# ownzonefeng/pytorch-distributed-training-example

Hardware: AMD Instinct MI355X
Metric: images/sec (whole node) ResNet-50 DDP at 1/2/4/8 MI355X; scaling efficiency (higher is better)
Workload: dtype bf16; 1 GPU; model=resnet50, global_batch=1024, per_gpu_batch=1024, image_size=224, parallelism=dp1, grad_accum=1, impl=ours, graph=False, precision=bf16, bucket_cap_mb=auto, comm_hook=none, reducer_active=True, pg_size=1, pg_backend=nccl, deterministic=False, full=False

## Files before the change

### pytorch_distributed_training_example_amd/config.py

```python
from __future__ import annotations

import os


class _Switches:
    __slots__ = ("disable_native", "conv1x1", "conv1x1_ours", "conv1x1_prefer", "conv1x1_override",
                 "conv1x1_table", "conv1x1_dump", "conv1x1_s2", "conv3x3", "conv3x3_wgrad", "conv3x3_s2", "conv_stem",
                 "conv_bn_stats", "bn_bwd_stats", "res_masked", "stem_bwd_fused", "stem_bn_wgrad", "stem_bn_stats", "stem_pool_wgrad", "wgrad_splitk", "slice_sum",
                 "subsample_native", "linear_splitk", "fused_addln", "embedding_native", "linear_epilogue",
                 "bwd_fused", "bwd_fused_shapes", "bwd_alg", "alg_glo", "bwd_alg_min_m", "z3_virtual", "bwd_alg_first", "ds_alg", "bn2_defer", "bn_apply_gemm_k", "strided_bstats", "gap_native", "sub_out",
                 "fp8_fused_gelu", "fp8_weight_multi", "fp8_cast_colsum", "fp8_ln", "wgrad_stream_m",
                 "dropout_fused")

    def __init__(self):
        self.reload()

    def reload(self) -> "_Switches":
        e = os.environ.get

        def on(name: str, default: str = "1") -> bool:
            return e(name, default) != "0"

        self.disable_native = e("PDT_DISABLE_NATIVE", "0") == "1"
        self.conv1x1 = e("PDT_CONV1X1", "auto")
# ... 2 lines not shown
        ov = e("PDT_CONV1X1_OVERRIDE", "")
        self.conv1x1_override = dict(p.split("=", 1) for p in ov.replace("+", ";").split(";") if "=" in p)
        self.conv1x1_table = on("PDT_CONV1X1_TABLE")
        self.conv1x1_dump = e("PDT_CONV1X1_DUMP") or None
        self.conv1x1_s2 = e("PDT_CONV1X1_S2", "1") == "1"
        self.conv3x3 = e("PDT_CONV3X3", "ours")
        self.conv3x3_wgrad = e("PDT_CONV3X3_WGRAD", "ours")
        self.conv3x3_s2 = e("PDT_CONV3X3_S2", "ours")
        self.conv_stem = e("PDT_CONV_STEM", "ours")
        self.conv_bn_stats = on("PDT_CONV_BN_STATS")
        self.bn_bwd_stats = on("PDT_BN_BWD_STATS")
        self.res_masked = on("PDT_RES_MASKED")
        self.stem_bwd_fused = on("PDT_STEM_BWD_FUSED")
        self.stem_bn_wgrad = on("PDT_STEM_BN_WGRAD")
        self.stem_bn_stats = on("PDT_STEM_BN_STATS")
        self.stem_pool_wgrad = on("PDT_STEM_POOL_WGRAD")
        self.wgrad_splitk = on("PDT_WGRAD_SPLITK")
        self.slice_sum = on("PDT_SLICE_SUM")
        self.subsample_native = on("PDT_SUBSAMPLE_NATIVE")
        self.linear_splitk = on("PDT_LINEAR_SPLITK")
        self.fused_addln = on("PDT_FUSED_ADDLN")
        self.embedding_native = on("PDT_EMBEDDING_NATIVE")
        self.linear_epilogue = e("PDT_LINEAR_EPILOGUE", "auto")
        self.bwd_fused = on("PDT_BWD_FUSED")
        self.bwd_fused_shapes = tuple(tuple(int(v) for v in t.split("x")) for t in
                                      e("PDT_BWD_FUSED_SHAPES", "256x64").split(",") if "x" in t)
        self.bwd_alg = int(e("PDT_BWD_ALG", "2"))
        self.bwd_alg_min_m = int(e("PDT_BWD_ALG_MIN_M", "50176"))
        self.alg_glo = on("PDT_ALG_GLO", "1")
        self.z3_virtual = int(e("PDT_Z3_VIRTUAL", "2"))
        self.bwd_alg_first = on("PDT_BWD_ALG_FIRST", "1")
        self.ds_alg = int(e("PDT_DS_ALG", "512"))
        self.bn2_defer = on("PDT_BN2_DEFER", "0")
        self.bn_apply_gemm_k = int(e("PDT_BN_APPLY_GEMM_K", "128"))
        self.strided_bstats = on("PDT_STRIDED_BSTATS")
        self.gap_native = on("PDT_GAP_NATIVE")
        self.sub_out = on("PDT_SUB_OUT")
        self.fp8_fused_gelu = on("PDT_FP8_FUSED_GELU")
        self.fp8_weight_multi = on("PDT_FP8_WEIGHT_MULTI")
        self.fp8_cast_colsum = on("PDT_FP8_CAST_COLSUM")
        self.fp8_ln = on("PDT_FP8_LN")
        self.wgrad_stream_m = int(e("PDT_WGRAD_STREAM_M", "0"))
        self.dropout_fused = on("PDT_DROPOUT_FUSED")
        return self


SW = _Switches()
```

### pytorch_distributed_training_example_amd/csrc/binding.cpp

```cpp
#include <torch/extension.h>
#include <ATen/hip/HIPContext.h>

#include <cstring>
#include <map>
#include <vector>

#include "fp8_pack.h"
#include "launchers.h"

namespace {

using at::Tensor;

hipStream_t stream() { return at::hip::getCurrentHIPStream().stream(); }

int dcode(const Tensor& t) {
  if (t.scalar_type() == at::kFloat) return 0;
  if (t.scalar_type() == at::kBFloat16) return 1;
  TORCH_CHECK(false, "pdt: unsupported dtype ", t.scalar_type(), " (fp32 / bf16 only)");
}

void check_cuda(const Tensor& t, const char* name) {
  TORCH_CHECK(t.is_cuda(), "pdt: ", name, " must be a GPU tensor");
}
// ... 2291 lines not shown
  m.doc() = "gfx950 HIP kernels for pytorch_distributed_training_example_amd";
  m.def("sgd", &sgd);
  m.def("adam", &adam);
  m.def("adadelta", &adadelta);
  m.def("lars", &lars);
  m.def("lamb", &lamb);
  m.def("layerwise_chunks", &layerwise_chunks);
  m.def("amp_unscale", &amp_unscale);
  m.def("amp_update", &amp_update);
  m.def("mt_scale", &mt_scale);
  m.def("mt_copy", &mt_copy);
  m.def("l2norm_sq", &l2norm_sq);
  m.def("clip_coef", &clip_coef);
  m.def("bn_tune", [](int variant, int target_blocks, int u_fwd, int u_bwd) {
    if (pdt_bn_tune(variant, target_blocks, u_fwd, u_bwd) != 0)
      throw py::value_error("bn_tune: variant must be 0 (keep), 3 (in-kernel finalize) or 5 (finalize kernel), got " +
                            std::to_string(variant));
  }, py::arg("variant") = 0, py::arg("target_blocks") = 0, py::arg("u_fwd") = 0, py::arg("u_bwd") = 0);
  m.def("bn_fwd_train", &bn_fwd_train, py::arg("x"), py::arg("res"), py::arg("weight"), py::arg("bias"),
        py::arg("running_mean"), py::arg("running_var"), py::arg("momentum"), py::arg("eps"), py::arg("relu"),
        py::arg("res_ab") = py::none(), py::arg("apply") = true);
  m.def("bn_fwd_eval", &bn_fwd_eval);
  m.def("bn_relu_maxpool_fwd", &bn_relu_maxpool_fwd);
  m.def("bn_relu_maxpool_fwd_parts", &bn_relu_maxpool_fwd_parts);
  m.def("maxpool3s2_bwd", &maxpool3s2_bwd);
  m.def("conv1x1_gemm", &conv1x1_gemm, py::arg("a"), py::arg("b"), py::arg("out"), py::arg("acc"), py::arg("stats"),
        py::arg("c_in") = py::none(), py::arg("c_mask") = py::none(), py::arg("bn_x") = py::none(),
        py::arg("bn_mask") = py::none(), py::arg("bn_mean") = py::none(), py::arg("c_stride") = 0,
        py::arg("c_H") = 0, py::arg("c_W") = 0, py::arg("a_coef") = py::none(), py::arg("bn_sum_only") = false,
        py::arg("no_store") = false);
  m.def("conv1x1_probe", [](int probe) { pdt_conv1x1_probe(probe); });
  m.def("conv1x1_persist", [](int mode) { return pdt_conv1x1_persist(mode); },
        "1x1 GEMM persistence mode (0 off, 1 measured kinds, 2 all, -1 env default); returns the previous mode");
  m.def("conv1x1_last_persistent", []() { return pdt_conv1x1_last_persistent(); },
        "which kernel the last 1x1 GEMM call launched: 0 one tile per workgroup, else the persistent kernel's waves "
        "per workgroup (+256 statistics-only, +512 APPLY)");
  m.def("conv3x3_opt", [](int v) { return pdt_conv3x3_opt(v); },
        "3x3 conv variant bits (csrc/kernels/conv3x3.hip conv3x3_opt; -1 env default); returns the previous value");
  m.def("weight_prep", &weight_prep);
  m.def("bn_tiles_fused", [](int on) { pdt_bn_tiles_fused(on); });
  m.def("maxpool_bwd_v2", [](int on) { pdt_maxpool_bwd_v2(on); });
  m.def("pool_fwd_contig", [](int on) { pdt_pool_fwd_contig(on); });
  m.def("bn_apply_wgs", [](int n) { pdt_bn_apply_wgs(n); });
  m.def("bn_row_wgs", [](int n) { pdt_bn_row_wgs(n); });
  m.def("gap_bwd", &gap_bwd, py::arg("g"), py::arg("H"), py::arg("W"), py::arg("bn_x") = py::none(),
        py::arg("bn_mask") = py::none(), py::arg("bn_mean") = py::none(), py::arg("bn_sum_only") = false);
  m.def("conv1x1_gemm_apply", &conv1x1_gemm_apply, py::arg("a"), py::arg("b"), py::arg("res"), py::arg("ab"),
        py::arg("rab") = py::none(), py::arg("a_coef") = py::none());
  m.def("bn_bwd_train_tiles", &bn_bwd_train_tiles);
  m.def("maxpool3s2_bwd_bn", &maxpool3s2_bwd_bn);
  m.def("maxpool3s2_bwd_bn_coef", &maxpool3s2_bwd_bn_coef, py::arg("dy"), py::arg("code"), py::arg("x"),
        py::arg("weight"), py::arg("mean"), py::arg("invstd"), py::arg("need_dgamma"), py::arg("write_dz") = true);
  m.def("slice_sum", &slice_sum);
  m.def("subsample_gather", &subsample_gather);
  m.def("subsample_scatter_add", &subsample_scatter_add);
  m.def("bn_fwd_train_tiles", &bn_fwd_train_tiles, py::arg("x"), py::arg("part"), py::arg("res"), py::arg("weight"),
        py::arg("bias"), py::arg("running_mean"), py::arg("running_var"), py::arg("momentum"), py::arg("eps"),
        py::arg("relu"), py::arg("res_ab") = py::none(), py::arg("apply") = true, py::arg("sub") = 0);
  m.def("conv3x3s1_fwd", &conv3x3s1_fwd);
  m.def("conv3x3s1_fwd_stats", &conv3x3s1_fwd_stats);
  m.def("conv3x3s1_fwd_bnbwd", &conv3x3s1_fwd_bnbwd);
  m.def("conv3x3_flip", &conv3x3_flip);
  m.def("conv3x3s2_fwd", &conv3x3s2_fwd);
  m.def("conv3x3s2_wgrad", &conv3x3s2_wgrad);
  m.def("conv3x3s2_dgrad", &conv3x3s2_dgrad, py::arg("dy"), py::arg("wf"), py::arg("H"), py::arg("W"),
        py::arg("bn_x") = py::none(), py::arg("bn_mask") = py::none(), py::arg("bn_mean") = py::none());
// ... 93 lines not shown
```

### pytorch_distributed_training_example_amd/csrc/kernels/conv1x1.hip

```cpp
#include "../common.h"
#include "../launchers.h"
#include "../tile_stats.h"

#include <stdlib.h>

using namespace pdt;

namespace {

typedef __bf16 bf16x8 __attribute__((ext_vector_type(8)));
typedef float f4 __attribute__((ext_vector_type(4)));
#define PDT_LDS __attribute__((address_space(3)))

__device__ __attribute__((aligned(256))) uint4 g_gemm_zero[16];
__device__ __attribute__((aligned(256))) uint4 g_gemm_ones[16] = {
    {0x3f803f80u, 0x3f803f80u, 0x3f803f80u, 0x3f803f80u}, {0x3f803f80u, 0x3f803f80u, 0x3f803f80u, 0x3f803f80u},
    {0x3f803f80u, 0x3f803f80u, 0x3f803f80u, 0x3f803f80u}, {0x3f803f80u, 0x3f803f80u, 0x3f803f80u, 0x3f803f80u},
    {0x3f803f80u, 0x3f803f80u, 0x3f803f80u, 0x3f803f80u}, {0x3f803f80u, 0x3f803f80u, 0x3f803f80u, 0x3f803f80u},
    {0x3f803f80u, 0x3f803f80u, 0x3f803f80u, 0x3f803f80u}, {0x3f803f80u, 0x3f803f80u, 0x3f803f80u, 0x3f803f80u},
    {0x3f803f80u, 0x3f803f80u, 0x3f803f80u, 0x3f803f80u}, {0x3f803f80u, 0x3f803f80u, 0x3f803f80u, 0x3f803f80u},
    {0x3f803f80u, 0x3f803f80u, 0x3f803f80u, 0x3f803f80u}, {0x3f803f80u, 0x3f803f80u, 0x3f803f80u, 0x3f803f80u},
    {0x3f803f80u, 0x3f803f80u, 0x3f803f80u, 0x3f803f80u}, {0x3f803f80u, 0x3f803f80u, 0x3f803f80u, 0x3f803f80u},
    {0x3f803f80u, 0x3f803f80u, 0x3f803f80u, 0x3f803f80u}, {0x3f803f80u, 0x3f803f80u, 0x3f803f80u, 0x3f803f80u}};
__device__ uint8_t g_mask_ones[16] = {
// ... 310 lines not shown
      v.z = (uint32_t)f2bf(z[4]) | ((uint32_t)f2bf(z[5]) << 16);
      v.w = (uint32_t)f2bf(z[6]) | ((uint32_t)f2bf(z[7]) << 16);
    }
    if constexpr (BSTATS) {
      bn_bwd_accum8(v, xbv[it], bmkv[it], bmu, bs1, bs2);
      v = mask8(v, bmkv[it]);
    }
    if (!ok) continue;
    if constexpr (STATS) rs8_add(rst, v);
    if constexpr (APPLY) {
      if (!(probe & 32)) ap.mask[off >> 3] = (uint8_t)amb;
    }
    if constexpr (!NOST) {
      if (probe & 1) continue;
      if constexpr (NT) {
        const u32x4 t = {v.x, v.y, v.z, v.w};
        __builtin_nontemporal_store(t, reinterpret_cast<u32x4*>(Y + off));
      } else {
        *reinterpret_cast<uint4*>(Y + off) = v;
      }
    }
  }
  }

  if constexpr (BSTATS)
    bn_bwd_tile_store<BN, Cf::kWaves>(bs1, bs2, reinterpret_cast<float*>(lds), bs.part, (M + BM - 1) / BM, mt, N, n0);
  if constexpr (STATS) {
    __syncthreads();
    rs8_tile_store<BN, Cf::kWaves>(rst, kst, reinterpret_cast<float*>(lds), part, min(BM, M - m0), (M + BM - 1) / BM,
                                   mt, N, n0);
  }
}

template <class Cf, int HV = 0>
struct PL {
  static constexpr int kStgOff = 2 * Cf::kSlot;
  static constexpr int kFull = Cf::BM * Cf::kEpiStride;
  static constexpr int kHalves = HV > 0 ? HV : (kStgOff + kFull <= 152 * 1024 ? 1 : 2);
  static_assert(Cf::WM % kHalves == 0, "a part is whole wave rows");
  static constexpr int kStg = kFull / kHalves;
  static constexpr int kRed0 = Cf::kWaves * (Cf::BN / 8) * 16 * 4, kRed1 = Cf::kWaves * 2 * Cf::BN * 4;
  static constexpr int kRed = kRed0 > kRed1 ? kRed0 : kRed1;
  static constexpr int kArea = kStg > kRed ? kStg : kRed;
  static constexpr int kLds = 3 * Cf::kSlot > kStgOff + kArea ? 3 * Cf::kSlot : kStgOff + kArea;
  static constexpr int kOcc = (160 * 1024) / kLds;
  static constexpr int kMinWaves = kOcc * Cf::kThreads / 256 > 0 ? kOcc * Cf::kThreads / 256 : 1;
  static_assert(kLds <= 160 * 1024 && kFull % kHalves == 0, "LDS");
};

__device__ __attribute__((aligned(256))) uint4 g_gemm_sink[1024];
__device__ uint8_t g_mask_sink[1024];

__device__ __forceinline__ void dma16a(const void* src, char* lds_wave_base) {
  const uint32_t m0 = __builtin_amdgcn_readfirstlane((uint32_t)(uintptr_t)(PDT_LDS const char*)lds_wave_base);
  asm volatile("s_mov_b32 m0, %1\n\ts_nop 0\n\tglobal_load_lds_dwordx4 %0, off" ::"v"(src), "s"(m0) : "memory");
}
template <int N>
__device__ __forceinline__ void wait_vmn() {
  static_assert(N >= 0 && N < 64, "vmcnt");
  __builtin_amdgcn_s_waitcnt((N & 15) | (7 << 4) | (15 << 8) | ((N >> 4) << 14));
}

template <class Cf, bool ACC, bool STATS, bool BSTATS, bool ATR, bool APPLY, bool STR, bool NOST = false, int HV = 0>
__global__ __launch_bounds__(Cf::kThreads, (PL<Cf, HV>::kMinWaves)) void conv1x1p_kernel(
    const uint16_t* __restrict__ A, const uint16_t* __restrict__ B, uint16_t* Y, const uint16_t* Cin,
    const uint8_t* __restrict__ Cmask, float* __restrict__ part, int M, int K, int N, BnSrc bs, CGeom cg,
    const float* __restrict__ acoef, ApArgs ap) {
  static_assert(!(APPLY && (ACC || STATS || BSTATS)), "APPLY is a forward epilogue of its own");
  static_assert(!STR || ACC, "STR: a strided accumulate source");
  static_assert(!NOST || (STATS && !ACC && !BSTATS && !APPLY), "NOST: the statistics-only forward");
  using L = PL<Cf, HV>;
  constexpr int BM = Cf::BM, BN = Cf::BN, kG = Cf::kG, kHalves = L::kHalves;
  constexpr int WROWS = BM / Cf::WM, WCOLS = BN / Cf::WN;
  extern __shared__ __attribute__((aligned(16))) char lds[];
  const int tid = threadIdx.x, lane = tid & 63, wid = __builtin_amdgcn_readfirstlane(tid >> 6);
  const int wm = wid % Cf::WM, wn = wid / Cf::WM;
  const int ntn = N / BN, T = (M + BM - 1) / BM, total = T * ntn;
  const int G = gridDim.x, xg = blockIdx.x % 8, jg = blockIdx.x / 8, gx = (G - xg + 7) / 8;
  const int c_lo = (int)((int64_t)total * xg / 8), c_hi = (int)((int64_t)total * (xg + 1) / 8);
  int tile = c_lo + jg;
  if (tile >= c_hi) return;
  const int S = K / Cf::BK;
  char* const stg = lds + L::kStgOff;

  const int sub = lane >> 2, p = lane & 3;
  auto aoff_of = [&](int m0, int i) {
    const int r = (wid * Cf::kALd + i) * 16 + sub;
    return m0 + r < M ? (m0 + r) * K + chk64(r, p) * 8 : -1;
  };
  auto boff_of = [&](int n0, int j) {
    const int r = (wid * Cf::kBLd + j) * 16 + sub;
    return (n0 + r) * K + chk64(r, p) * 8;
  };
  int aoff[Cf::kALd], boff[Cf::kBLd];
  auto issue = [&](int s, int slot_i) {
    char* slot = lds + slot_i * Cf::kSlot;
    const int ko = s * Cf::BK;
#pragma unroll
    for (int i = 0; i < Cf::kALd; ++i)
      dma16a(aoff[i] >= 0 ? (const void*)(A + (aoff[i] + ko)) : (const void*)g_gemm_zero, slot + (wid * Cf::kALd + i) * 1024);
#pragma unroll
    for (int j = 0; j < Cf::kBLd; ++j) dma16a(B + (boff[j] + ko), slot + Cf::kABytes + (wid * Cf::kBLd + j) * 1024);
  };

  float* const ctab = reinterpret_cast<float*>(lds + L::kLds);
  float* const atab = ctab + (ATR ? 2 * K : 0);
  if constexpr (ATR) {
    for (int i = tid; i < 2 * K; i += Cf::kThreads) ctab[i] = acoef[i];
    __syncthreads();
  }
  constexpr int kChunks = BN / 8;
  constexpr int kRowStep = Cf::kThreads / kChunks, kIt = BM / kRowStep;
  constexpr int kItH = kIt / kHalves;
  constexpr int kB = (ACC && BSTATS) ? (Cf::kWaves >= 16 ? 2 : (kItH >= 8 ? kItH / 2 : kItH))
                     : (APPLY && kItH > 2) ? 2 : kItH;
  constexpr int kStores = NOST ? 0 : kIt * (APPLY ? 2 : 1);
// ... 82 lines not shown
    const int next = tile + gx;
    const bool has_next = next < c_hi;
    if (has_next) {
      mt = next / ntn; n0 = (next % ntn) * BN; m0 = mt * BM;
#pragma unroll
      for (int i = 0; i < Cf::kALd; ++i) aoff[i] = aoff_of(m0, i);
#pragma unroll
      for (int j = 0; j < Cf::kBLd; ++j) boff[j] = boff_of(n0, j);
      issue(0, 0);
      if (S > 1) issue(1, 1);
    }

    RowStats8 rst;
    float kst = 0.f;
    float bs1[8], bs2[8], bmu[8];
    if constexpr (APPLY) {
      if (cur_n0 != tab_n0) {
        if (tid < BN) {
          atab[tid] = ap.ab[cur_n0 + tid];
          atab[BN + tid] = ap.ab[N + cur_n0 + tid];
          atab[2 * BN + tid] = ap.rab ? ap.rab[cur_n0 + tid] : 1.f;
          atab[3 * BN + tid] = ap.rab ? ap.rab[N + cur_n0 + tid] : 0.f;
        }
        tab_n0 = cur_n0;
      }
    }
    if constexpr (BSTATS) {
      *reinterpret_cast<float4*>(bmu) = *reinterpret_cast<const float4*>(bs.mean + cur_n0 + c * 8);
      *reinterpret_cast<float4*>(bmu + 4) = *reinterpret_cast<const float4*>(bs.mean + cur_n0 + c * 8 + 4);
#pragma unroll
      for (int k = 0; k < 8; ++k) { bs1[k] = 0.f; bs2[k] = 0.f; }
    }
#pragma unroll
    for (int hv = 0; hv < kHalves; ++hv) {
      constexpr int kWH = Cf::WM / kHalves;
      if (wm / kWH == hv) {
#pragma unroll
        for (int i = 0; i < Cf::kMB; ++i)
#pragma unroll
          for (int j = 0; j < Cf::kNB; ++j) {
            const int ml = (wm % kWH) * WROWS + i * 16 + lrow;
            const int cl = wn * WCOLS + j * 16 + 4 * lchk;
            *reinterpret_cast<uint2*>(stg + ml * Cf::kEpiStride + cl * 2) = pk[i][j];
          }
      }
      asm volatile("s_waitcnt lgkmcnt(0)" ::: "memory");
      __builtin_amdgcn_s_barrier();
      asm volatile("" ::: "memory");
      if constexpr (STATS) {
        if (hv == 0) {
          rs8_init(rst, *reinterpret_cast<const uint4*>(stg + (tid % kChunks) * 16));
          if (tid < BN) kst = __uint_as_float((uint32_t)*reinterpret_cast<const uint16_t*>(stg + tid * 2) << 16);
        }
      }
#pragma unroll
      for (int h = hv * kItH; h < (hv + 1) * kItH; h += kB) {
        uint4 cv[kB], xbv[kB];
        unsigned cmk[kB], bmkv[kB];
        bool okv[kB];
#pragma unroll
        for (int it = 0; it < kB; ++it) {
          const int m = cur_m0 + r0 + kRowStep * (h + it);
          const bool ok = m < M;
          okv[it] = ok;
          const int mc = ok ? m : M - 1;
          const int64_t off = (int64_t)mc * N + cur_n0 + c * 8;
          if constexpr (BSTATS) {
            xbv[it] = *reinterpret_cast<const uint4*>(bx_base + off * bx_scale);
            const unsigned b8 = bm_base[(off >> 3) * bm_scale];
            bmkv[it] = ok ? b8 : 0u;
          }
          if constexpr (APPLY) cv[it] = *reinterpret_cast<const uint4*>(Cin + off);
          if constexpr (ACC) {
            const unsigned mk = cm_base[(off >> 3) * cm_scale];
            if constexpr (STR) {
              const int w = mc % cg.W, t = mc / cg.W, hh = t % cg.H, n = t / cg.H;
              const bool on = hh % cg.s == 0 && w % cg.s == 0;
              const int64_t co = on ? ((int64_t)(n * cg.Hs + hh / cg.s) * cg.Ws + w / cg.s) * N : 0;
              cv[it] = *reinterpret_cast<const uint4*>(Cin + co + cur_n0 + c * 8);
              cmk[it] = on ? mk : 0u;
            } else {
              cv[it] = *reinterpret_cast<const uint4*>(Cin + off);
// ... 24 lines not shown
            v.w = (uint32_t)f2bf(a8[6]) | ((uint32_t)f2bf(a8[7]) << 16);
          }
          unsigned amb = 0;
          if constexpr (APPLY) {
            const uint32_t w[4] = {v.x, v.y, v.z, v.w}, rw[4] = {cv[it].x, cv[it].y, cv[it].z, cv[it].w};
            uint32_t o[4];
            asm volatile("" ::: "memory");
#pragma unroll
            for (int q = 0; q < 2; ++q) {
              float fa[4], fb[4], fra[4], frb[4], z[4];
              *reinterpret_cast<float4*>(fa) = *reinterpret_cast<const float4*>(atab + c * 8 + 4 * q);
              *reinterpret_cast<float4*>(fb) = *reinterpret_cast<const float4*>(atab + BN + c * 8 + 4 * q);
              *reinterpret_cast<float4*>(fra) = *reinterpret_cast<const float4*>(atab + 2 * BN + c * 8 + 4 * q);
              *reinterpret_cast<float4*>(frb) = *reinterpret_cast<const float4*>(atab + 3 * BN + c * 8 + 4 * q);
#pragma unroll
              for (int k = 0; k < 4; ++k) {
                const uint32_t wz = w[2 * q + (k >> 1)], wr = rw[2 * q + (k >> 1)];
                const float zf = __uint_as_float(k & 1 ? wz & 0xffff0000u : wz << 16);
                const float rf = __uint_as_float(k & 1 ? wr & 0xffff0000u : wr << 16);
                float t = zf * fa[k] + fb[k];
                t += ap.rab ? rf * fra[k] + frb[k] : rf;
                amb |= (t > 0.f ? 1u : 0u) << (4 * q + k);
                z[k] = t > 0.f ? t : 0.f;
              }
              o[2 * q] = (uint32_t)f2bf(z[0]) | ((uint32_t)f2bf(z[1]) << 16);
              o[2 * q + 1] = (uint32_t)f2bf(z[2]) | ((uint32_t)f2bf(z[3]) << 16);
            }
            v = make_uint4(o[0], o[1], o[2], o[3]);
          }
          if constexpr (BSTATS) {
            bn_bwd_accum8(v, xbv[it], bmkv[it], bmu, bs1, bs2);
            v = mask8(v, bmkv[it]);
          }
          if constexpr (STATS) {
            if (ok) rs8_add(rst, v);
          }
          if constexpr (!NOST) {
            uint4* yp = ok ? reinterpret_cast<uint4*>(Y + off) : g_gemm_sink + tid;
            *yp = v;
          }
          if constexpr (APPLY) {
            uint8_t* mp = ok ? ap.mask + (off >> 3) : g_mask_sink + tid;
            *mp = (uint8_t)amb;
          }
        }
      }
      __builtin_amdgcn_s_barrier();
      asm volatile("" ::: "memory");
    }
    if constexpr (BSTATS)
      bn_bwd_tile_store<BN, Cf::kWaves>(bs1, bs2, reinterpret_cast<float*>(stg), bs.part, T, cur_mt, N, cur_n0);
    if constexpr (STATS)
      rs8_tile_store<BN, Cf::kWaves>(rst, kst, reinterpret_cast<float*>(stg), part, min(BM, M - cur_m0), T, cur_mt, N,
                                     cur_n0);
    if constexpr (BSTATS || STATS) {
      asm volatile("s_waitcnt lgkmcnt(0)" ::: "memory");
      __builtin_amdgcn_s_barrier();
      asm volatile("" ::: "memory");
    }
    if (!has_next) break;
    tile = next;
    first = false;
  }
  wait_vmn<0>();
}

int g_persist = -1;

inline int persist_mode() {
  if (g_persist < 0) {
    const char* e = getenv("PDT_CONV1X1_PERSIST");
    g_persist = (e && e[0]) ? (int)strtol(e, nullptr, 10) : 1;
    if (g_persist < 0 || g_persist > 2) g_persist = 1;
  }
  return g_persist;
}

int g_last_persistent = 0;

template <class Cf, bool ACC, bool STATS, bool BSTATS, bool ATR, bool APPLY, bool STR, bool NOST = false, int HV = 0>
int launch_p(const uint16_t* a, const uint16_t* b, uint16_t* y, const uint16_t* c, const uint8_t* cm, float* part, int M,
             int K, int N, const BnSrc& bs, const CGeom& cg, hipStream_t s, const float* acoef, const ApArgs& ap) {
  using L = PL<Cf, HV>;
  static bool attr = false;
  constexpr int kTab = APPLY ? 4 * Cf::BN * 4 : 0;
  constexpr int kMaxLds = L::kLds + (ATR ? 2 * 512 * 4 : 0) + kTab;
  static_assert(kMaxLds <= 160 * 1024, "LDS");
  if (!attr) {
    if (hipFuncSetAttribute(
            reinterpret_cast<const void*>(&conv1x1p_kernel<Cf, ACC, STATS, BSTATS, ATR, APPLY, STR, NOST, HV>),
            hipFuncAttributeMaxDynamicSharedMemorySize, kMaxLds) != hipSuccess)
      return -3;
    attr = true;
  }
  const int lds = L::kLds + (ATR ? 2 * K * 4 : 0) + kTab;
  const int64_t total = (int64_t)(M + Cf::BM - 1) / Cf::BM * (N / Cf::BN);
  const int occ = (160 * 1024) / lds > 0 ? (160 * 1024) / lds : 1;
  int64_t grid = 256 * (int64_t)occ;
  if (grid > total) grid = total;
  hipLaunchKernelGGL((conv1x1p_kernel<Cf, ACC, STATS, BSTATS, ATR, APPLY, STR, NOST, HV>), dim3((unsigned)grid),
                     dim3(Cf::kThreads), lds, s, a, b, y, c, cm, part, M, K, N, bs, cg, acoef, ap);
  g_last_persistent = Cf::kWaves | (NOST ? 256 : 0) | (APPLY ? 512 : 0);
  return 0;
}

constexpr int kMaxATRK = 512;

template <class Cf, bool ACC, bool STATS, bool NT, bool BSTATS, bool ATR = false, bool APPLY = false, bool STR = false,
          bool NOST = false>
int launch_nt(const uint16_t* a, const uint16_t* b, uint16_t* y, const uint16_t* c, const uint8_t* cm, float* part,
              int M, int K, int N, const BnSrc& bs, const CGeom& cg, hipStream_t s, const float* acoef = nullptr,
              const ApArgs& ap = ApArgs{}) {
  static bool attr = false;
  constexpr int kMaxLds = Cf::kLds + (ATR ? 2 * kMaxATRK * 4 : 0);
  if (!attr) {
    if (hipFuncSetAttribute(
            reinterpret_cast<const void*>(&conv1x1_kernel<Cf, ACC, STATS, NT, BSTATS, ATR, APPLY, STR, NOST>),
            hipFuncAttributeMaxDynamicSharedMemorySize, kMaxLds) != hipSuccess)
      return -3;
    attr = true;
  }
  if (ATR && K > kMaxATRK) return -1;
  const int lds = Cf::kLds + (ATR ? 2 * K * 4 : 0);
  const int64_t grid = (int64_t)(M + Cf::BM - 1) / Cf::BM * (N / Cf::BN);
  ApArgs apx = ap;
  apx.probe = g_probe;
  if constexpr (!NT) {
    constexpr int kHV = (APPLY && !ATR && Cf::kWaves == 8 && Cf::WM == 4) ? 4 : 0;
    constexpr bool kMeasured = (Cf::kWaves >= 16 && !ACC && !ATR && !APPLY) || (APPLY && !ATR && kHV == 4);
    const int pm = persist_mode();
    if ((pm == 2 || (pm == 1 && kMeasured)) && g_probe == 0 && !ap.a2 &&
        grid >= 2 * 256 * (int64_t)((160 * 1024) / PL<Cf, kHV>::kLds))
      return launch_p<Cf, ACC, STATS, BSTATS, ATR, APPLY, STR, NOST, kHV>(a, b, y, c, cm, part, M, K, N, bs, cg, s, acoef,
                                                                          apx);
  }
  hipLaunchKernelGGL((conv1x1_kernel<Cf, ACC, STATS, NT, BSTATS, ATR, APPLY, STR, NOST>), dim3((unsigned)grid),
                     dim3(Cf::kThreads), lds, s, a, b, y, c, cm, part, M, K, N, bs, cg, acoef, apx);
  g_last_persistent = 0;
  return 0;
}

template <class Cf, bool ACC, bool STATS, bool BSTATS = false>
int launch(const uint16_t* a, const uint16_t* b, uint16_t* y, const uint16_t* c, const uint8_t* cm, float* part, int M,
           int K, int N, const BnSrc& bs, const CGeom& cg, hipStream_t s, const ApArgs& ap = ApArgs{}) {
  if constexpr (ACC)
    if (cg.s) return launch_nt<Cf, ACC, STATS, false, BSTATS, false, false, true>(a, b, y, c, cm, part, M, K, N, bs, cg, s,
                                                                                  nullptr, ap);
  if constexpr (STATS && !ACC && !BSTATS)
    if (ap.nostore)
      return launch_nt<Cf, false, true, false, false, false, false, false, true>(a, b, y, c, cm, part, M, K, N, bs, cg, s,
                                                                                 nullptr, ap);
  return launch_nt<Cf, ACC, STATS, false, BSTATS>(a, b, y, c, cm, part, M, K, N, bs, cg, s, nullptr, ap);
}

using GXWide = G1<256, 4, 4>;
using GWide = G1<128, 4, 2>;
using GNarrow = G1<64, 4, 1>;
using GXWide2 = G1<256, 2, 4>;
inline bool w2_on() {
  static const int v = [] {
    const char* e = getenv("PDT_CONV1X1_W2");
    return (e && e[0]) ? (int)strtol(e, nullptr, 10) : 0;
  }();
  return v != 0;
}

template <class Cf>
int dispatch(const uint16_t* a, const uint16_t* b, uint16_t* y, const uint16_t* c, const uint8_t* cm, float* part,
             int M, int K, int N, const BnSrc& bs, const CGeom& cg, hipStream_t s, const float* acoef = nullptr,
             const ApArgs& ap = ApArgs{}) {
  if ((c && part) || (cm && !c) || (part && bs.part) || (cg.s && (!c || cm))) return -1;
  if (acoef) {
    if (c || bs.part) return -1;
    if (part) return launch_nt<Cf, false, true, false, false, true>(a, b, y, c, cm, part, M, K, N, bs, cg, s, acoef);
    return launch_nt<Cf, false, false, false, false, true>(a, b, y, c, cm, part, M, K, N, bs, cg, s, acoef);
  }
  if (bs.part) {
    if (!bs.mean) return -1;
    if (c) return launch<Cf, true, false, true>(a, b, y, c, cm, part, M, K, N, bs, cg, s);
    return launch<Cf, false, false, true>(a, b, y, c, cm, part, M, K, N, bs, cg, s);
  }
  if (c) return launch<Cf, true, false>(a, b, y, c, cm, part, M, K, N, bs, cg, s);
  if (part) return launch<Cf, false, true>(a, b, y, c, cm, part, M, K, N, bs, cg, s, ap);
  return launch<Cf, false, false>(a, b, y, c, cm, part, M, K, N, bs, cg, s);
}

}

extern "C" {

int pdt_conv1x1_tile_rows() { return 256; }

void pdt_conv1x1_probe(int probe) { g_probe = probe; }

int pdt_conv1x1_persist(int mode) {
  const int old = persist_mode();
  g_persist = mode < 0 ? -1 : (mode > 2 ? 2 : mode);
  return old;
}

int pdt_conv1x1_last_persistent() { return g_last_persistent; }

int pdt_conv1x1_gemm(const uint16_t* a, const uint16_t* b, uint16_t* y, const uint16_t* c, const uint8_t* cm,
                     float* part, int M, int K, int N, const uint16_t* bn_x, const uint8_t* bn_mask,
                     const float* bn_mean, float* bn_part, int c_s, int c_H, int c_W, const float* acoef,
                     hipStream_t s, int nostore) {
  ApArgs ap{};
  ap.nostore = nostore && part && !c && !acoef && !bn_part ? 1 : 0;
  if (nostore && !ap.nostore) return -1;
  if (M < 1 || K < 32 || K % 32 != 0 || N < 64 || N % 64 != 0) return -1;
  if ((int64_t)M * (K > N ? K : N) >= ((int64_t)1 << 31) || (int64_t)N * K >= ((int64_t)1 << 31)) return -2;
  const BnSrc bs{bn_x, bn_mask, bn_mean, bn_part};
  CGeom cg{0, 1, 1, 1, 1};
  if (c_s > 0) {
    if (c_H < 1 || c_W < 1 || M % (c_H * c_W) != 0) return -1;
    cg = CGeom{c_s, c_H, c_W, (c_H - 1) / c_s + 1, (c_W - 1) / c_s + 1};
  }
  if (w2_on() && N % 256 == 0 && K >= 256 && !c && !acoef && !bs.part && !(g_probe & 64))
    return dispatch<GXWide2>(a, b, y, c, cm, part, M, K, N, bs, cg, s, acoef, ap);
  if (N % 256 == 0 && (int64_t)((M + 255) / 256) * (N / 256) >= 2048 && !(g_probe & 64) && !c && !acoef)
    return dispatch<GXWide>(a, b, y, c, cm, part, M, K, N, bs, cg, s, acoef, ap);
  if (N % 128 == 0 && !(g_probe & 8) && !small_grid_narrow((int64_t)((M + 255) / 256) * (N / 128)))
    return dispatch<GWide>(a, b, y, c, cm, part, M, K, N, bs, cg, s, acoef, ap);
  return dispatch<GNarrow>(a, b, y, c, cm, part, M, K, N, bs, cg, s, acoef, ap);
}

int pdt_conv1x1_gemm_seg(const uint16_t* a1, int k1, const uint16_t* a2, int k2, int rep2, const uint16_t* b,
                         uint16_t* y, int M, int N, const uint16_t* bn_x, const uint8_t* bn_mask, const float* bn_mean,
                         float* bn_part, hipStream_t s) {
  const int K = k1 + rep2 * k2 + 32;
// ... 51 lines not shown
```

### pytorch_distributed_training_example_amd/csrc/launchers.h

```cpp
#pragma once
#include <hip/hip_runtime.h>
#include <stdint.h>

extern "C" {

int pdt_amp_unscale(int n, void* const* g, const int64_t* numel, int dtype, const float* inv_scale, float* found_inf,
                    hipStream_t s);
int pdt_amp_update(float* scale, int* growth_tracker, const float* found_inf, float growth, float backoff,
                   int interval, hipStream_t s);
int pdt_mt_scale(int n, void* const* x, const int64_t* numel, int dtype, const float* scale_ptr, float scale,
                 hipStream_t s);
int pdt_mt_copy(int n, void* const* src, void* const* dst, const int64_t* numel, int sdt, int ddt,
                const float* scale_ptr, float scale, hipStream_t s);
int pdt_l2norm_sq(int n, void* const* x, const int64_t* numel, int dtype, float* out, hipStream_t s);
int pdt_clip_coef(const float* sumsq, float max_norm, float* coef, float* norm, hipStream_t s);

int pdt_attn_fwd(const uint16_t* q, const int64_t* qs, const uint16_t* k, const int64_t* ks, const uint16_t* v,
                 const int64_t* vs, uint16_t* o, const int64_t* os, float* lse, int B, int H, int T, int Dh,
                 int causal, float scale, hipStream_t s);
int pdt_attn_bwd(const uint16_t* dout, const int64_t* dos, const uint16_t* q, const int64_t* qs, const uint16_t* k,
                 const int64_t* ks, const uint16_t* v, const int64_t* vs, const uint16_t* o, const int64_t* os,
                 const float* lse, float* delta, uint16_t* dq, uint16_t* dk, uint16_t* dv, const int64_t* gs, int B,
                 int H, int T, int Dh, int causal, float scale, hipStream_t s);
int pdt_attn_fwd_drop(const uint16_t* q, const int64_t* qs, const uint16_t* k, const int64_t* ks, const uint16_t* v,
// ... 61 lines not shown
int pdt_maxpool_bn_parts(int N, int H);
int pdt_maxpool3s2_bwd_bn(const uint16_t* dy, const uint8_t* code, uint16_t* dz, int N, int H, int W, int C,
                          const uint16_t* x, const float* gamma, const float* mean, const float* invstd, uint16_t* dx,
                          float* dgamma, float* dbeta, float* part, float* ws, hipStream_t s);
int pdt_maxpool3s2_bwd_bn_coef(const uint16_t* dy, const uint8_t* code, uint16_t* dz, int N, int H, int W, int C,
                               const uint16_t* x, const float* gamma, const float* mean, const float* invstd,
                               float* coef, float* dgamma, float* dbeta, float* part, float* ws, hipStream_t s);
int pdt_bn_sync_fwd_stats(const uint16_t* x, int64_t M, int C, float* stats, float* count, float* ws,
                          unsigned* counters, hipStream_t s);
int pdt_bn_sync_fwd_merge(const float* gathered, int W, int C, const float* gamma, const float* beta,
                          float* running_mean, float* running_var, float momentum, float eps, float* mean,
                          float* invstd, float* ab, int64_t* ntot, hipStream_t s);
int pdt_bn_apply_coef(const uint16_t* x, const uint16_t* res, const float* ab, int64_t M, int C, int relu,
                      uint16_t* y, uint8_t* mask, hipStream_t s);
int pdt_bn_sync_bwd_sums(const uint16_t* dy, const uint16_t* x, const uint8_t* mask, const float* mean, int64_t M,
                         int C, int relu, float* sums, float* ws, unsigned* counters, hipStream_t s);
int pdt_bn_sync_bwd_merge(const float* gathered, int W, int rank, int C, const float* gamma, const float* invstd,
                          const int64_t* ntot, float* coef, float* dgamma, float* dbeta, hipStream_t s);
int pdt_bn_bwd_apply_coef(const uint16_t* dy, const uint16_t* x, const uint8_t* mask, const float* mean,
                          const float* coef, int64_t M, int C, int relu, int has_res, uint16_t* dx, uint16_t* dres,
                          hipStream_t s);

int pdt_bn_alg_fix_s2(float* part, int T, const float* wg, const uint16_t* W, int C4, int CW, hipStream_t s);
int pdt_bn_alg_ds_part(float* part, const float* s1, const float* mean, const float* wg, const uint16_t* W, int C4,
                       int CW, hipStream_t s);
int pdt_bn_alg_small_gemm(const uint16_t* W, const uint16_t* Wt, const float* coef, const float* wg, float* G,
                          float* BWG, int C4, int CW, hipStream_t s);
int pdt_bn_alg_assemble(const uint16_t* W, const float* coef, const float* mean, const float* G, const float* wg,
                        const float* BWG, uint16_t* bcat, uint16_t* dW, int C4, int CW, int rep, hipStream_t s);

int pdt_conv1x1_tile_rows();
void pdt_conv1x1_probe(int probe);
int pdt_conv1x1_persist(int mode);
int pdt_conv1x1_last_persistent();
int pdt_conv1x1_gemm(const uint16_t* a, const uint16_t* b, uint16_t* y, const uint16_t* c, const uint8_t* cm,
                     float* part, int M, int K, int N, const uint16_t* bn_x, const uint8_t* bn_mask,
                     const float* bn_mean, float* bn_part, int c_s, int c_H, int c_W, const float* acoef,
                     hipStream_t s, int nostore);
int pdt_conv1x1_gemm_seg(const uint16_t* a1, int k1, const uint16_t* a2, int k2, int rep2, const uint16_t* b,
                         uint16_t* y, int M, int N, const uint16_t* bn_x, const uint8_t* bn_mask,
                         const float* bn_mean, float* bn_part, hipStream_t s);
int pdt_conv1x1_gemm_apply(const uint16_t* a, const uint16_t* b, uint16_t* y, const uint16_t* res, const float* ab,
                           const float* rab, uint8_t* mask, int M, int K, int N, const float* acoef, hipStream_t s);

int pdt_conv1x1_bwd_fused_ok(int C4, int CW);
int pdt_conv1x1_bwd_fused_grid(int M, int C4, int CW);
int pdt_conv1x1_bwd_fused(const uint16_t* dy, const uint16_t* z, const uint8_t* mz, const float* mean, const float* A,
                          const float* B, const float* D, const uint16_t* wt, const uint16_t* xa, const uint16_t* bx,
                          const uint8_t* bm, const float* bmean, float* bpart, const float* xcoef, uint8_t* mask_out,
                          uint16_t* dxa, uint16_t* dw, float* ws, int M, int C4, int CW, hipStream_t s);
void pdt_conv1x1_bwd_fused_tune(int grid);

int64_t pdt_conv1x1_wgrad_ws_floats(int M, int Ci, int Co, int* nsplit_out);
int pdt_conv1x1_wgrad(const uint16_t* x, const uint16_t* dy, uint16_t* dw, float* ws, int M, int Ci, int Co,
                      hipStream_t s);
int64_t pdt_conv1x1_wgrad_seg_ws_floats(int M, int Ci, int co1, int co2, int* rows_out);
int pdt_conv1x1_wgrad_seg(const uint16_t* x, const uint16_t* dy1, int co1, const uint16_t* dy2, int co2, float* out,
                          float* ws, int M, int Ci, hipStream_t s);
void pdt_conv1x1_wgrad_tune(int target_wgs, int variant, int interleave);

int pdt_conv3x3s1_fwd(const uint16_t* x, const uint16_t* w, uint16_t* y, int N, int H, int W, int Ci, int Co,
                      hipStream_t s);
int pdt_conv3x3s1_stats_tile_rows(int N, int H, int W, int Ci, int Co);
int pdt_conv3x3s1_bnbwd_tile_rows(int N, int H, int W, int Ci, int Co);
int pdt_conv3x3s1_fwd_stats(const uint16_t* x, const uint16_t* w, uint16_t* y, float* part, int N, int H, int W,
                            int Ci, int Co, hipStream_t s);
// ... 173 lines not shown
```

### pytorch_distributed_training_example_amd/csrc/tile_stats.h

```cpp
#pragma once
#include <hip/hip_runtime.h>
#include <stdint.h>

namespace pdt {

template <int BM, int BN, int THREADS, int STRIDE>
__device__ __forceinline__ void tile_bn_stats(const char* tile, float* red, int nvalid, float* __restrict__ part,
                                              int mt, int T, int N, int n0) {
  constexpr int kGroups = THREADS / (BN / 2);
  constexpr int kRows = BM / kGroups;
  static_assert(BM % kGroups == 0, "row groups");
  const int tid = threadIdx.x;
  const int cp = tid % (BN / 2), g = tid / (BN / 2);
  const char* col = tile + cp * 4;
  float s0 = 0.f, s1 = 0.f;
#pragma unroll 8
  for (int rr = 0; rr < kRows; ++rr) {
    const int r = g * kRows + rr;
    const uint32_t v = *reinterpret_cast<const uint32_t*>(col + r * STRIDE);
    if (r < nvalid) { s0 += __uint_as_float(v << 16); s1 += __uint_as_float(v & 0xffff0000u); }
  }
  red[g * BN + 2 * cp] = s0;
  red[g * BN + 2 * cp + 1] = s1;
  __syncthreads();
// ... 65 lines not shown
  };
  static_assert(kChunks >= 8, "xor_add distances");
#pragma unroll
  for (int j = 0; j < 4; ++j) {
    t.s[j] = pdt_f2{xr(t.s[j].x), xr(t.s[j].y)};
    t.q[j] = pdt_f2{xr(t.q[j].x), xr(t.q[j].y)};
  }
  if (lane < kChunks) {
    float* r = red + (wid * kChunks + lane) * 16;
#pragma unroll
    for (int j = 0; j < 4; ++j) {
      r[2 * j] = t.s[j].x; r[2 * j + 1] = t.s[j].y;
      r[8 + 2 * j] = t.q[j].x; r[8 + 2 * j + 1] = t.q[j].y;
    }
  }
  __syncthreads();
  if (tid < BN) {
    const int c = tid >> 3, j = tid & 7;
    float S = 0.f, Q = 0.f;
#pragma unroll
    for (int w = 0; w < WAVES; ++w) {
      S += red[(w * kChunks + c) * 16 + j];
      Q += red[(w * kChunks + c) * 16 + 8 + j];
    }
    const float n = (float)nvalid;
    part[(int64_t)mt * N + n0 + tid] = fmaf(n, K, S);
    part[((int64_t)T + mt) * N + n0 + tid] = fmaxf(Q - S * S / n, 0.f);
  }
}

template <int BN, int WAVES>
constexpr int rs8_tile_store_lds() { return WAVES * (BN / 8) * 16 * 4; }

struct BnSrc {
  const uint16_t* x;
  const uint8_t* mask;
  const float* mean;
  float* part;
};

__device__ __forceinline__ void bn_bwd_accum8(uint4 v, uint4 xb, unsigned mk, const float (&mu)[8], float (&s1)[8],
                                              float (&s2)[8]) {
  const uint32_t w[4] = {v.x, v.y, v.z, v.w}, xw[4] = {xb.x, xb.y, xb.z, xb.w};
#pragma unroll
  for (int k = 0; k < 8; ++k) {
    const uint32_t gb = k & 1 ? (w[k >> 1] & 0xffff0000u) : (w[k >> 1] << 16);
    const uint32_t xv = k & 1 ? (xw[k >> 1] & 0xffff0000u) : (xw[k >> 1] << 16);
    const float g = (mk >> k) & 1u ? __uint_as_float(gb) : 0.f;
    s1[k] += g;
    s2[k] += g * (__uint_as_float(xv) - mu[k]);
  }
}

__device__ __forceinline__ uint4 mask8(uint4 v, unsigned mk) {
  uint32_t w[4] = {v.x, v.y, v.z, v.w};
#pragma unroll
  for (int k = 0; k < 4; ++k) {
    const uint32_t lo = (mk >> (2 * k)) & 1u ? 0x0000ffffu : 0u, hi = (mk >> (2 * k + 1)) & 1u ? 0xffff0000u : 0u;
    w[k] &= lo | hi;
  }
  return make_uint4(w[0], w[1], w[2], w[3]);
}

template <int BN, int WAVES>
__device__ __forceinline__ void bn_bwd_tile_store(float (&s1)[8], float (&s2)[8], float* red, float* __restrict__ part,
                                                  int T, int mt, int N, int n0) {
// ... 31 lines not shown
```

Baseline: 16690 images/sec.

## Compute 1x1 GEMM batch-norm statistics from accumulator registers in persistent kernel

New measurement: 16790 images/sec (median of 6 runs). No clear change (+0.7%).

```diff
diff --git a/pytorch_distributed_training_example_amd/config.py b/pytorch_distributed_training_example_amd/config.py
--- a/pytorch_distributed_training_example_amd/config.py
+++ b/pytorch_distributed_training_example_amd/config.py
@@ -58,7 +58,7 @@
         self.bwd_alg_first = on("PDT_BWD_ALG_FIRST", "1")
         self.ds_alg = int(e("PDT_DS_ALG", "512"))
         self.bn2_defer = on("PDT_BN2_DEFER", "0")
-        self.bn_apply_gemm_k = int(e("PDT_BN_APPLY_GEMM_K", "128"))
+        self.bn_apply_gemm_k = int(e("PDT_BN_APPLY_GEMM_K", "256"))
         self.strided_bstats = on("PDT_STRIDED_BSTATS")
         self.gap_native = on("PDT_GAP_NATIVE")
         self.sub_out = on("PDT_SUB_OUT")
diff --git a/pytorch_distributed_training_example_amd/csrc/binding.cpp b/pytorch_distributed_training_example_amd/csrc/binding.cpp
--- a/pytorch_distributed_training_example_amd/csrc/binding.cpp
+++ b/pytorch_distributed_training_example_amd/csrc/binding.cpp
@@ -2347,6 +2347,9 @@
   m.def("conv1x1_probe", [](int probe) { pdt_conv1x1_probe(probe); });
   m.def("conv1x1_persist", [](int mode) { return pdt_conv1x1_persist(mode); },
         "1x1 GEMM persistence mode (0 off, 1 measured kinds, 2 all, -1 env default); returns the previous mode");
+  m.def("conv1x1_stats_mode", [](int mode) { return pdt_conv1x1_stats_mode(mode); },
+        "statistics of the persistent 16-wave 1x1 GEMM tile (0 staged reduction, 1 from the accumulator registers); "
+        "returns the previous mode");
   m.def("conv1x1_last_persistent", []() { return pdt_conv1x1_last_persistent(); },
         "which kernel the last 1x1 GEMM call launched: 0 one tile per workgroup, else the persistent kernel's waves "
         "per workgroup (+256 statistics-only, +512 APPLY)");
diff --git a/pytorch_distributed_training_example_amd/csrc/kernels/conv1x1.hip b/pytorch_distributed_training_example_amd/csrc/kernels/conv1x1.hip
--- a/pytorch_distributed_training_example_amd/csrc/kernels/conv1x1.hip
+++ b/pytorch_distributed_training_example_amd/csrc/kernels/conv1x1.hip
@@ -366,7 +366,7 @@
   }
 }
 
-template <class Cf, int HV = 0>
+template <class Cf, int HV = 0, int XM = 0>
 struct PL {
   static constexpr int kStgOff = 2 * Cf::kSlot;
   static constexpr int kFull = Cf::BM * Cf::kEpiStride;
@@ -375,8 +375,12 @@
   static constexpr int kStg = kFull / kHalves;
   static constexpr int kRed0 = Cf::kWaves * (Cf::BN / 8) * 16 * 4, kRed1 = Cf::kWaves * 2 * Cf::BN * 4;
   static constexpr int kRed = kRed0 > kRed1 ? kRed0 : kRed1;
-  static constexpr int kArea = kStg > kRed ? kStg : kRed;
-  static constexpr int kLds = 3 * Cf::kSlot > kStgOff + kArea ? 3 * Cf::kSlot : kStgOff + kArea;
+  static constexpr int kXch = XM ? reg_tile_stats_lds<Cf::WM, Cf::WN, Cf::kMB, Cf::kNB>() : 0;
+  static constexpr int kArea = XM == 1 ? kXch : XM == 2 ? kStg : (kStg > kRed ? kStg : kRed);
+  static constexpr int kXchOff = XM == 2 ? kStgOff + kArea : kStgOff;
+  static constexpr int kEnd = XM == 2 ? kXchOff + kXch : kStgOff + kArea;
+  static constexpr int kLds = 3 * Cf::kSlot > kEnd ? 3 * Cf::kSlot : kEnd;
+  static_assert(XM != 1 || kXch <= Cf::kSlot, "the exchange fits ring slot 2");
   static constexpr int kOcc = (160 * 1024) / kLds;
   static constexpr int kMinWaves = kOcc * Cf::kThreads / 256 > 0 ? kOcc * Cf::kThreads / 256 : 1;
   static_assert(kLds <= 160 * 1024 && kFull % kHalves == 0, "LDS");
@@ -395,15 +399,17 @@
   __builtin_amdgcn_s_waitcnt((N & 15) | (7 << 4) | (15 << 8) | ((N >> 4) << 14));
 }
 
-template <class Cf, bool ACC, bool STATS, bool BSTATS, bool ATR, bool APPLY, bool STR, bool NOST = false, int HV = 0>
-__global__ __launch_bounds__(Cf::kThreads, (PL<Cf, HV>::kMinWaves)) void conv1x1p_kernel(
+template <class Cf, bool ACC, bool STATS, bool BSTATS, bool ATR, bool APPLY, bool STR, bool NOST = false, int HV = 0,
+          bool RG = false>
+__global__ __launch_bounds__(Cf::kThreads, (PL<Cf, HV, RG ? (NOST ? 1 : 2) : 0>::kMinWaves)) void conv1x1p_kernel(
     const uint16_t* __restrict__ A, const uint16_t* __restrict__ B, uint16_t* Y, const uint16_t* Cin,
     const uint8_t* __restrict__ Cmask, float* __restrict__ part, int M, int K, int N, BnSrc bs, CGeom cg,
     const float* __restrict__ acoef, ApArgs ap) {
   static_assert(!(APPLY && (ACC || STATS || BSTATS)), "APPLY is a forward epilogue of its own");
   static_assert(!STR || ACC, "STR: a strided accumulate source");
   static_assert(!NOST || (STATS && !ACC && !BSTATS && !APPLY), "NOST: the statistics-only forward");
-  using L = PL<Cf, HV>;
+  static_assert(!RG || (STATS && !ACC && !BSTATS && !APPLY && !ATR), "RG: the statistics forward");
+  using L = PL<Cf, HV, RG ? (NOST ? 1 : 2) : 0>;
   constexpr int BM = Cf::BM, BN = Cf::BN, kG = Cf::kG, kHalves = L::kHalves;
   constexpr int WROWS = BM / Cf::WM, WCOLS = BN / Cf::WN;
   extern __shared__ __attribute__((aligned(16))) char lds[];
@@ -416,6 +422,7 @@
   if (tile >= c_hi) return;
   const int S = K / Cf::BK;
   char* const stg = lds + L::kStgOff;
+  float* const xch = reinterpret_cast<float*>(lds + L::kXchOff);
 
   const int sub = lane >> 2, p = lane & 3;
   auto aoff_of = [&](int m0, int i) {
@@ -564,7 +571,7 @@
       for (int k = 0; k < 8; ++k) { bs1[k] = 0.f; bs2[k] = 0.f; }
     }
 #pragma unroll
-    for (int hv = 0; hv < kHalves; ++hv) {
+    for (int hv = 0; hv < (NOST && RG ? 0 : kHalves); ++hv) {
       constexpr int kWH = Cf::WM / kHalves;
       if (wm / kWH == hv) {
 #pragma unroll
@@ -579,7 +586,7 @@
       asm volatile("s_waitcnt lgkmcnt(0)" ::: "memory");
       __builtin_amdgcn_s_barrier();
       asm volatile("" ::: "memory");
-      if constexpr (STATS) {
+      if constexpr (STATS && !RG) {
         if (hv == 0) {
           rs8_init(rst, *reinterpret_cast<const uint4*>(stg + (tid % kChunks) * 16));
           if (tid < BN) kst = __uint_as_float((uint32_t)*reinterpret_cast<const uint16_t*>(stg + tid * 2) << 16);
@@ -670,8 +677,15 @@
             bn_bwd_accum8(v, xbv[it], bmkv[it], bmu, bs1, bs2);
             v = mask8(v, bmkv[it]);
           }
-          if constexpr (STATS) {
+          if constexpr (STATS && !RG) {
             if (ok) rs8_add(rst, v);
+          }
+          if constexpr (RG) {
+            constexpr int kEvery = kIt / Cf::kNB;
+            static_assert(kIt % Cf::kNB == 0, "a statistics slice every kEvery rows");
+            if ((h + it) % kEvery == 0)
+              reg_tile_stats_slice<Cf::WM, Cf::WN, Cf::kMB, Cf::kNB>(pk, (h + it) / kEvery, wm, wn, xch,
+                                                                     min(BM, M - cur_m0));
           }
           if constexpr (!NOST) {
             uint4* yp = ok ? reinterpret_cast<uint4*>(Y + off) : g_gemm_sink + tid;
@@ -688,10 +702,18 @@
     }
     if constexpr (BSTATS)
       bn_bwd_tile_store<BN, Cf::kWaves>(bs1, bs2, reinterpret_cast<float*>(stg), bs.part, T, cur_mt, N, cur_n0);
-    if constexpr (STATS)
+    if constexpr (RG) {
+      if constexpr (NOST) {
+#pragma unroll
+        for (int j = 0; j < Cf::kNB; ++j)
+          reg_tile_stats_slice<Cf::WM, Cf::WN, Cf::kMB, Cf::kNB>(pk, j, wm, wn, xch, min(BM, M - cur_m0));
+      }
+      reg_tile_stats_store<Cf::WM, Cf::WN, Cf::kMB, Cf::kNB>(xch, part, min(BM, M - cur_m0), T, cur_mt, N, cur_n0);
+    }
+    if constexpr (STATS && !RG)
       rs8_tile_store<BN, Cf::kWaves>(rst, kst, reinterpret_cast<float*>(stg), part, min(BM, M - cur_m0), T, cur_mt, N,
                                      cur_n0);
-    if constexpr (BSTATS || STATS) {
+    if constexpr (BSTATS || (STATS && !RG)) {
       asm volatile("s_waitcnt lgkmcnt(0)" ::: "memory");
       __builtin_amdgcn_s_barrier();
       asm volatile("" ::: "memory");
@@ -716,17 +738,20 @@
 
 int g_last_persistent = 0;
 
-template <class Cf, bool ACC, bool STATS, bool BSTATS, bool ATR, bool APPLY, bool STR, bool NOST = false, int HV = 0>
+int g_stats_mode = 1;
+
+template <class Cf, bool ACC, bool STATS, bool BSTATS, bool ATR, bool APPLY, bool STR, bool NOST = false, int HV = 0,
+          bool RG = false>
 int launch_p(const uint16_t* a, const uint16_t* b, uint16_t* y, const uint16_t* c, const uint8_t* cm, float* part, int M,
              int K, int N, const BnSrc& bs, const CGeom& cg, hipStream_t s, const float* acoef, const ApArgs& ap) {
-  using L = PL<Cf, HV>;
+  using L = PL<Cf, HV, RG ? (NOST ? 1 : 2) : 0>;
   static bool attr = false;
   constexpr int kTab = APPLY ? 4 * Cf::BN * 4 : 0;
   constexpr int kMaxLds = L::kLds + (ATR ? 2 * 512 * 4 : 0) + kTab;
   static_assert(kMaxLds <= 160 * 1024, "LDS");
   if (!attr) {
     if (hipFuncSetAttribute(
-            reinterpret_cast<const void*>(&conv1x1p_kernel<Cf, ACC, STATS, BSTATS, ATR, APPLY, STR, NOST, HV>),
+            reinterpret_cast<const void*>(&conv1x1p_kernel<Cf, ACC, STATS, BSTATS, ATR, APPLY, STR, NOST, HV, RG>),
             hipFuncAttributeMaxDynamicSharedMemorySize, kMaxLds) != hipSuccess)
       return -3;
     attr = true;
@@ -736,7 +761,7 @@
   const int occ = (160 * 1024) / lds > 0 ? (160 * 1024) / lds : 1;
   int64_t grid = 256 * (int64_t)occ;
   if (grid > total) grid = total;
-  hipLaunchKernelGGL((conv1x1p_kernel<Cf, ACC, STATS, BSTATS, ATR, APPLY, STR, NOST, HV>), dim3((unsigned)grid),
+  hipLaunchKernelGGL((conv1x1p_kernel<Cf, ACC, STATS, BSTATS, ATR, APPLY, STR, NOST, HV, RG>), dim3((unsigned)grid),
                      dim3(Cf::kThreads), lds, s, a, b, y, c, cm, part, M, K, N, bs, cg, acoef, ap);
   g_last_persistent = Cf::kWaves | (NOST ? 256 : 0) | (APPLY ? 512 : 0);
   return 0;
@@ -768,9 +793,14 @@
     constexpr bool kMeasured = (Cf::kWaves >= 16 && !ACC && !ATR && !APPLY) || (APPLY && !ATR && kHV == 4);
     const int pm = persist_mode();
     if ((pm == 2 || (pm == 1 && kMeasured)) && g_probe == 0 && !ap.a2 &&
-        grid >= 2 * 256 * (int64_t)((160 * 1024) / PL<Cf, kHV>::kLds))
+        grid >= 2 * 256 * (int64_t)((160 * 1024) / PL<Cf, kHV>::kLds)) {
+      if constexpr (STATS && !ACC && !BSTATS && !ATR && !APPLY && Cf::kWaves >= 16 && Cf::WM == 4)
+        if (g_stats_mode == 1)
+          return launch_p<Cf, ACC, STATS, BSTATS, ATR, APPLY, STR, NOST, kHV, true>(a, b, y, c, cm, part, M, K, N, bs, cg,
+                                                                                    s, acoef, apx);
       return launch_p<Cf, ACC, STATS, BSTATS, ATR, APPLY, STR, NOST, kHV>(a, b, y, c, cm, part, M, K, N, bs, cg, s, acoef,
                                                                           apx);
+    }
   }
   hipLaunchKernelGGL((conv1x1_kernel<Cf, ACC, STATS, NT, BSTATS, ATR, APPLY, STR, NOST>), dim3((unsigned)grid),
                      dim3(Cf::kThreads), lds, s, a, b, y, c, cm, part, M, K, N, bs, cg, acoef, apx);
@@ -834,6 +864,12 @@
 int pdt_conv1x1_persist(int mode) {
   const int old = persist_mode();
   g_persist = mode < 0 ? -1 : (mode > 2 ? 2 : mode);
+  return old;
+}
+
+int pdt_conv1x1_stats_mode(int mode) {
+  const int old = g_stats_mode;
+  g_stats_mode = mode != 0 ? 1 : 0;
   return old;
 }
 
diff --git a/pytorch_distributed_training_example_amd/csrc/launchers.h b/pytorch_distributed_training_example_amd/csrc/launchers.h
--- a/pytorch_distributed_training_example_amd/csrc/launchers.h
+++ b/pytorch_distributed_training_example_amd/csrc/launchers.h
@@ -117,6 +117,7 @@
 int pdt_conv1x1_tile_rows();
 void pdt_conv1x1_probe(int probe);
 int pdt_conv1x1_persist(int mode);
+int pdt_conv1x1_stats_mode(int mode);
 int pdt_conv1x1_last_persistent();
 int pdt_conv1x1_gemm(const uint16_t* a, const uint16_t* b, uint16_t* y, const uint16_t* c, const uint8_t* cm,
                      float* part, int M, int K, int N, const uint16_t* bn_x, const uint8_t* bn_mask,
diff --git a/pytorch_distributed_training_example_amd/csrc/tile_stats.h b/pytorch_distributed_training_example_amd/csrc/tile_stats.h
--- a/pytorch_distributed_training_example_amd/csrc/tile_stats.h
+++ b/pytorch_distributed_training_example_amd/csrc/tile_stats.h
@@ -121,6 +121,91 @@
 template <int BN, int WAVES>
 constexpr int rs8_tile_store_lds() { return WAVES * (BN / 8) * 16 * 4; }
 
+template <bool MASK, int MB>
+__device__ __forceinline__ float reg_m2(const float (&x)[MB], float mean, int lrow, int nw) {
+  float q = 0.f;
+#pragma unroll
+  for (int i = 0; i < MB; ++i) {
+    const float d = x[i] - mean;
+    if constexpr (MASK) q = i * 16 + lrow < nw ? fmaf(d, d, q) : q;
+    else q = fmaf(d, d, q);
+  }
+  return row16_sum(q);
+}
+
+template <int WM, int WN, int MB, int NB>
+constexpr int reg_tile_stats_lds() { return WM * WN * NB * 16 * 2 * 4; }
+
+template <int WROWS>
+__device__ __forceinline__ int reg_wave_rows(int nvalid, int w) {
+  const int r = nvalid - w * WROWS;
+  return r < 0 ? 0 : (r > WROWS ? WROWS : r);
+}
+
+template <int WM, int WN, int MB, int NB>
+__device__ __forceinline__ void reg_tile_stats_slice(const uint2 (&pk)[MB][NB], int j, int wm, int wn, float* xch,
+                                                     int nvalid) {
+  constexpr int WROWS = MB * 16, WCOLS = NB * 16, kWaves = WM * WN;
+  int tid = threadIdx.x;
+  asm volatile("" : "+v"(tid));
+  const int lane = tid & 63, lrow = lane & 15, lchk = lane >> 4;
+  const int nw = reg_wave_rows<WROWS>(nvalid, wm);
+  const float inv_n = nw > 0 ? 1.f / (float)nw : 0.f;
+  float* const xs = xch + (wm + WM * wn) * WCOLS;
+  float x[4][MB];
+#pragma unroll
+  for (int i = 0; i < MB; ++i) {
+    x[0][i] = __uint_as_float(pk[i][j].x << 16); x[1][i] = __uint_as_float(pk[i][j].x & 0xffff0000u);
+    x[2][i] = __uint_as_float(pk[i][j].y << 16); x[3][i] = __uint_as_float(pk[i][j].y & 0xffff0000u);
+  }
+  float s[4], q[4];
+#pragma unroll
+  for (int e = 0; e < 4; ++e) {
+    float t = x[e][0];
+#pragma unroll
+    for (int i = 1; i < MB; ++i) t += x[e][i];
+    s[e] = row16_sum(t);
+  }
+  if (nw == WROWS) {
+#pragma unroll
+    for (int e = 0; e < 4; ++e) q[e] = reg_m2<false, MB>(x[e], s[e] * inv_n, lrow, nw);
+  } else {
+#pragma unroll
+    for (int e = 0; e < 4; ++e) q[e] = reg_m2<true, MB>(x[e], s[e] * inv_n, lrow, nw);
+  }
+  if (lrow == 0) {
+    *reinterpret_cast<float4*>(xs + j * 16 + 4 * lchk) = make_float4(s[0], s[1], s[2], s[3]);
+    *reinterpret_cast<float4*>(xs + kWaves * WCOLS + j * 16 + 4 * lchk) = make_float4(q[0], q[1], q[2], q[3]);
+  }
+}
+
+template <int WM, int WN, int MB, int NB>
+__device__ __forceinline__ void reg_tile_stats_store(const float* xch, float* __restrict__ part, int nvalid, int T,
+                                                     int mt, int N, int n0) {
+  constexpr int WROWS = MB * 16, WCOLS = NB * 16, BN = WN * WCOLS, kWaves = WM * WN;
+  asm volatile("s_waitcnt lgkmcnt(0)" ::: "memory");
+  __builtin_amdgcn_s_barrier();
+  asm volatile("" ::: "memory");
+  const int tid = threadIdx.x;
+  if (tid < BN) {
+    const float* src = xch + WM * (tid / WCOLS) * WCOLS + tid % WCOLS;
+    float n = (float)reg_wave_rows<WROWS>(nvalid, 0), S = src[0], M2 = src[kWaves * WCOLS];
+#pragma unroll
+    for (int w = 1; w < WM; ++w) {
+      const int nb = reg_wave_rows<WROWS>(nvalid, w);
+      if (nb > 0) {
+        const float fb = (float)nb, Sb = src[w * WCOLS], Mb = src[kWaves * WCOLS + w * WCOLS];
+        const float delta = Sb / fb - S / n;
+        M2 = M2 + Mb + delta * delta * (n * fb / (n + fb));
+        S += Sb;
+        n += fb;
+      }
+    }
+    part[(int64_t)mt * N + n0 + tid] = S;
+    part[((int64_t)T + mt) * N + n0 + tid] = M2;
+  }
+}
+
 struct BnSrc {
   const uint16_t* x;
   const uint8_t* mask;
```
